# UW-ACL/SCPToolbox.jl

Hardware: NVIDIA H100
Metric: SCP iterations/sec (batch) (higher is better)
Workload: dtype f64

## Files before the change

### scptoolbox.jl_b200/csrc/conic_debug.cu

```cuda
#include "../../include/scpb.h"
#include "conic_symbolic.h"

struct SplitSums {
    std::vector<double> part;
    std::vector<int> cnt, tgt, taken;
    explicit SplitSums(int nslot) : part((size_t)nslot, 0.0), cnt((size_t)nslot, 0), tgt((size_t)nslot, -1), taken((size_t)nslot, 0) {}
    bool add(const int *it, const std::vector<int> &info, double p, double *y)
    {
        if (!it[3]) { y[it[0]] -= p; return true; }
        const size_t q = (size_t)it[3] - 1;
        if (it[3] < 1 || 4 * q + 3 >= info.size()) return false;
        const int *e = &info[4 * q];
        const int sl = e[3];
        if (e[0] != it[0] || e[1] < 0 || e[2] > (int)part.size() || sl < e[1] || sl >= e[2]) return false;
        part[sl] = p;
        if (++cnt[e[1]] == e[2] - e[1]) {
            double acc = y[e[0]];
            for (int k = e[1]; k < e[2]; k++) acc -= part[k];
            y[e[0]] = acc;
            cnt[e[1]] = 0;
        }
        return true;
    }
    bool store(const int *it, double p, double *y)
    {
        if (!it[3]) { y[it[0]] -= p; return true; }
        const int sl = it[3] - 1;
        if (sl < 0 || sl >= (int)part.size() || tgt[sl] >= 0) return false;
        part[sl] = p; tgt[sl] = it[0];
        return true;
    }
    bool take(int t, int s0, int s1, double &acc, bool entry)
    {
        for (int k = s0; k < s1; k++) {
            if (k < 0 || k >= (int)part.size() || tgt[k] != t) return false;
            acc -= part[k];
            taken[k] += entry;
        }
        return true;
    }
    bool level_done()
    {
        bool ok = true;
        for (size_t k = 0; k < cnt.size(); k++) {
            if (cnt[k] || (tgt[k] >= 0 && taken[k] != 1)) ok = false;
            tgt[k] = -1; taken[k] = 0;
        }
        return ok;
    }
};

static bool phase_b_operands(SplitSums &split, const int *it, const int *cm, int nnzL, std::vector<double> &Y, double &e, double &d)
{
    e = Y[it[0]];
    if (!split.take(it[0], cm[0], cm[1], e, true)) return false;
    if (it[3] & 2) { d = e; return true; }
    d = Y[(size_t)nnzL + it[1]];
    if (!split.take(nnzL + it[1], cm[2], cm[3], d, false)) return false;
    Y[it[0]] = e;
    return true;
}

extern "C" int32_t scpb_debug_kkt_solve(int32_t n, int32_t p, int32_t m, const int32_t *A_rp, const int32_t *A_ci,
                                        const int32_t *G_rp, const int32_t *G_ci, int32_t l, int32_t nsoc,
                                        const int32_t *soc_dims, const int32_t *perm, const double *Av,
                                        const double *Gv, const double *wm, double delta, double delta_dyn,
                                        const double *rhs, double *sol, int64_t *info)
{
    ConeSymbolic S;
    static const int zero = 0;
    if (!cone_symbolic_build(S, n, p, m, A_rp, A_ci ? A_ci : &zero, G_rp, G_ci ? G_ci : &zero, l, nsoc, soc_dims, perm))
        return SCPB_ERR_ARG;
    const int nk = S.nk, ntgt = S.nnzL + nk;
    std::vector<double> Y(ntgt), Ls(S.nnzL + 1), invD(nk), v(nk);
    for (int t = 0; t < ntgt; t++) {
        double acc = delta * S.as_sign[t];
        if (S.as_src[t] >= 0) acc += Av[S.as_src[t]];
        for (int k = S.as_ptr[t]; k < S.as_ptr[t + 1]; k++) acc += Gv[S.as_a[k]] * Gv[S.as_b[k]] * wm[S.as_c[k]];
        Y[t] = acc;
    }
    SplitSums split(S.npart);
    int64_t nsplit = 0;
    for (int lv = 0; lv < S.nlevels; lv++) {
        const int R = S.fa_R[lv];
        for (int w = S.fa_lvl[lv]; w < S.fa_lvl[lv + 1]; w++) {
            const int *it = &S.fa_item[4 * (size_t)w];
            if (it[2] - it[1] > R * CONIC_FACTOR_PF) return SCPB_ERR_ARG;
            double part = 0.0;
            for (int k = it[1]; k < it[2]; k++) part += Y[S.ft_op[2 * (size_t)k]] * Ls[S.Lr_pos[S.ft_op[2 * (size_t)k + 1]]];
            if (!split.store(it, part, Y.data())) return SCPB_ERR_ARG;
            nsplit += it[3] != 0;
        }
        for (int w = S.fb_lvl[lv]; w < S.fb_lvl[lv + 1]; w++) {
            const int *it = &S.fb_item[4 * (size_t)w];
            double e, d;
            if (!phase_b_operands(split, it, &S.fb_cmb[4 * (size_t)w], S.nnzL, Y, e, d)) return SCPB_ERR_ARG;
            const double sgn = (it[3] & 1) ? 1.0 : -1.0;
            if (!(sgn * d > delta_dyn)) d = sgn * delta_dyn;
            if (it[3] & 2) invD[it[1]] = 1.0 / d;
            else Ls[it[0]] = e * (1.0 / d);
        }
        if (!split.level_done()) return SCPB_ERR_ARG;
    }
    for (int i = 0; i < nk; i++) v[S.iperm[i]] = rhs[i];
    std::vector<double> Lrow(S.nnzL + 1);
    for (int k = 0; k < S.nnzL; k++) Lrow[k] = Ls[S.Lr_pos[k]];
    for (int lv = 0; lv < S.nlevels; lv++) {
        const int R = S.fwp_R[lv];
        for (int w = S.fwp_lvl[lv]; w < S.fwp_lvl[lv + 1]; w++) {
            const int *it = &S.fwp_item[4 * (size_t)w];
            if (it[2] - it[1] > R * CONIC_SOLVE_PF) return SCPB_ERR_ARG;
            double part = 0.0;
            for (int k = it[1]; k < it[2]; k++) part += Lrow[k] * v[S.Lr_col[k]];
            if (!split.add(it, S.fwc_item, part, v.data())) return SCPB_ERR_ARG;
            nsplit += it[3] != 0;
        }
        if (!split.level_done()) return SCPB_ERR_ARG;
    }
    for (int i = 0; i < nk; i++) v[i] *= invD[i];
    for (int lv = S.nlevels - 1; lv >= 0; lv--) {
        const int R = S.bwp_R[lv];
        for (int w = S.bwp_lvl[lv]; w < S.bwp_lvl[lv + 1]; w++) {
            const int *it = &S.bwp_item[4 * (size_t)w];
            if (it[2] - it[1] > R * CONIC_SOLVE_PF) return SCPB_ERR_ARG;
            double part = 0.0;
            for (int k = it[1]; k < it[2]; k++) part += Ls[k] * v[S.L_ri[k]];
            if (!split.add(it, S.bwc_item, part, v.data())) return SCPB_ERR_ARG;
            nsplit += it[3] != 0;
        }
        if (!split.level_done()) return SCPB_ERR_ARG;
    }
    for (int i = 0; i < nk; i++) sol[i] = v[S.iperm[i]];
    if (info) { info[0] = S.nnzL; info[1] = S.nlevels; info[2] = S.factor_ops; info[3] = (int64_t)S.as_a.size(); info[4] = nsplit; }
    return SCPB_OK;
}

extern "C" int32_t scpb_debug_kkt_solve_sn(int32_t n, int32_t p, int32_t m, const int32_t *A_rp, const int32_t *A_ci,
                                           const int32_t *G_rp, const int32_t *G_ci, int32_t l, int32_t nsoc,
                                           const int32_t *soc_dims, const int32_t *perm, const double *Av,
                                           const double *Gv, const double *wm, double delta, double delta_dyn,
                                           const double *rhs, double *sol, int64_t *info)
{
    ConeSymbolic S;
    static const int zero = 0;
    if (!cone_symbolic_build(S, n, p, m, A_rp, A_ci ? A_ci : &zero, G_rp, G_ci ? G_ci : &zero, l, nsoc, soc_dims, perm))
        return SCPB_ERR_ARG;
    const int nk = S.nk, ntgt = S.nnzL + nk, ns = (int)S.sn_first.size();
    std::vector<double> P((size_t)S.sn_panel_size, 0.0), invD(nk), v(nk);
    for (int t = 0; t < ntgt; t++) {
        double acc = delta * S.as_sign[t];
        if (S.as_src[t] >= 0) acc += Av[S.as_src[t]];
        for (int k = S.as_ptr[t]; k < S.as_ptr[t + 1]; k++) acc += Gv[S.as_a[k]] * Gv[S.as_b[k]] * wm[S.as_c[k]];
        P[(size_t)S.sn_pos_of_target[t]] = acc;
    }
    for (int lv = 0; lv < S.sn_nlevels; lv++)
        for (int w_ = S.sn_lvl_ptr[lv]; w_ < S.sn_lvl_ptr[lv + 1]; w_++) {
            const int s = S.sn_lvl_nodes[w_], a = S.sn_first[s], w = S.sn_width[s], R = S.sn_nrows[s];
            double *Q = &P[(size_t)S.sn_panel_off[s]];
            for (int c = 0; c < w; c++) {
                double d = Q[c + (size_t)R * c];
                const double sgn = (double)S.as_sign[S.nnzL + a + c];
                if (!(sgn * d > delta_dyn)) d = sgn * delta_dyn;
                Q[c + (size_t)R * c] = d;
                invD[a + c] = 1.0 / d;
                for (int r = c + 1; r < R; r++) Q[r + (size_t)R * c] /= d;
                for (int c2 = c + 1; c2 < w; c2++) {
                    const double f = Q[c2 + (size_t)R * c] * d;
                    for (int r = c2; r < R; r++) Q[r + (size_t)R * c2] -= Q[r + (size_t)R * c] * f;
                }
            }
            int k = S.sn_upd_ptr[s];
            for (int y = 0; y < R - w; y++)
                for (int x = y; x < R - w; x++) {
                    double u = 0.0;
                    for (int c = 0; c < w; c++) u += Q[w + x + (size_t)R * c] * Q[c + (size_t)R * c] * Q[w + y + (size_t)R * c];
                    P[(size_t)S.sn_upd_dst[k++]] -= u;
                }
        }
    for (int i = 0; i < nk; i++) v[S.iperm[i]] = rhs[i];
    for (int lv = 0; lv < S.sn_nlevels; lv++)
        for (int w_ = S.sn_lvl_ptr[lv]; w_ < S.sn_lvl_ptr[lv + 1]; w_++) {
            const int s = S.sn_lvl_nodes[w_], w = S.sn_width[s], R = S.sn_nrows[s];
            const double *Q = &P[(size_t)S.sn_panel_off[s]];
            const int *rows = &S.sn_rows[S.sn_rows_ptr[s]];
            for (int c = 0; c < w; c++) {
                const double xc = v[rows[c]];
                for (int r = c + 1; r < R; r++) v[rows[r]] -= Q[r + (size_t)R * c] * xc;
            }
        }
    for (int i = 0; i < nk; i++) v[i] *= invD[i];
    for (int lv = S.sn_nlevels - 1; lv >= 0; lv--)
        for (int w_ = S.sn_lvl_ptr[lv]; w_ < S.sn_lvl_ptr[lv + 1]; w_++) {
            const int s = S.sn_lvl_nodes[w_], w = S.sn_width[s], R = S.sn_nrows[s];
            const double *Q = &P[(size_t)S.sn_panel_off[s]];
            const int *rows = &S.sn_rows[S.sn_rows_ptr[s]];
            for (int c = w - 1; c >= 0; c--) {
                double acc = v[rows[c]];
                for (int r = c + 1; r < R; r++) acc -= Q[r + (size_t)R * c] * v[rows[r]];
                v[rows[c]] = acc;
            }
        }
    for (int i = 0; i < nk; i++) sol[i] = v[S.iperm[i]];
    if (info) {
        info[0] = ns; info[1] = S.sn_nlevels; info[2] = S.sn_panel_size; info[3] = (int64_t)S.sn_upd_dst.size();
        int wmax = 0, rmax = 0;
        for (int s = 0; s < ns; s++) { wmax = std::max(wmax, S.sn_width[s]); rmax = std::max(rmax, S.sn_nrows[s]); }
        info[4] = wmax; info[5] = rmax; info[6] = S.nlevels; info[7] = S.nnzL;
    }
    (void)ns;
    return SCPB_OK;
}

extern "C" int32_t scpb_debug_kkt_solve_hy(int32_t n, int32_t p, int32_t m, const int32_t *A_rp, const int32_t *A_ci,
                                           const int32_t *G_rp, const int32_t *G_ci, int32_t l, int32_t nsoc,
                                           const int32_t *soc_dims, const int32_t *perm, const double *Av,
                                           const double *Gv, const double *wm, double delta, double delta_dyn,
                                           int32_t cut, const double *rhs, double *sol, int64_t *info)
{
    ConeSymbolic S;
    static const int zero = 0;
    if (!cone_symbolic_build(S, n, p, m, A_rp, A_ci ? A_ci : &zero, G_rp, G_ci ? G_ci : &zero, l, nsoc, soc_dims, perm))
        return SCPB_ERR_ARG;
    if (!cone_symbolic_build_hybrid(S, cut)) return SCPB_ERR_UNSUPPORTED;
    const int nk = S.nk, ntgt = S.nnzL + nk, nl = S.hy_nlevels;
    std::vector<double> Y(ntgt), Ls(S.nnzL + 1), invD(nk), v(nk);
    for (int t = 0; t < ntgt; t++) {
        double acc = delta * S.as_sign[t];
        if (S.as_src[t] >= 0) acc += Av[S.as_src[t]];
        for (int k = S.as_ptr[t]; k < S.as_ptr[t + 1]; k++) acc += Gv[S.as_a[k]] * Gv[S.as_b[k]] * wm[S.as_c[k]];
        Y[t] = acc;
    }
    SplitSums split(S.npart);
    for (int lv = 0; lv < nl; lv++) {
        const int R = S.hy_fa_R[lv];
        for (int w = S.hy_fa_lvl[lv]; w < S.hy_fa_lvl[lv + 1]; w++) {
            const int *it = &S.hy_fa_item[4 * (size_t)w];
            if (it[2] - it[1] > R * CONIC_FACTOR_PF) return SCPB_ERR_ARG;
            double part = 0.0;
            for (int k = it[1]; k < it[2]; k++) part += Y[S.hy_ft_op[2 * (size_t)k]] * Ls[S.Lr_pos[S.hy_ft_op[2 * (size_t)k + 1]]];
            if (!split.store(it, part, Y.data())) return SCPB_ERR_ARG;
        }
        for (int w = S.hy_fb_lvl[lv]; w < S.hy_fb_lvl[lv + 1]; w++) {
            const int *it = &S.hy_fb_item[4 * (size_t)w];
            double e, d;
            if (!phase_b_operands(split, it, &S.hy_fb_cmb[4 * (size_t)w], S.nnzL, Y, e, d)) return SCPB_ERR_ARG;
            if (it[3] & 4) continue;
            const double sgn = (it[3] & 1) ? 1.0 : -1.0;
            if (!(sgn * d > delta_dyn)) d = sgn * delta_dyn;
            if (it[3] & 2) invD[it[1]] = 1.0 / d;
            else Ls[it[0]] = e * (1.0 / d);
        }
        if (!split.level_done()) return SCPB_ERR_ARG;
    }
    auto ppos = [&](const int *d, int r, int c) { return r == c ? S.nnzL + d[0] + c : d[3] + c * (d[2] - 1) - (c * (c - 1)) / 2 + (r - c - 1); };
    for (int tl = 0; tl < S.hy_ntl; tl++)
        for (int q = S.hy_tl_ptr[tl]; q < S.hy_tl_ptr[tl + 1]; q++) {
            const int *d = &S.hy_desc[8 * (size_t)q];
            const int w = d[1], R = d[2];
            std::vector<double> Q((size_t)R * w, 0.0), dd(w);
            for (int c = 0; c < w; c++)
                for (int r = c; r < R; r++) Q[r + (size_t)R * c] = Y[ppos(d, r, c)];
            for (int c = 0; c < w; c++) {
                double piv = Q[c + (size_t)R * c];
                const double sgn = ((d[6] >> c) & 1) ? 1.0 : -1.0;
                if (!(sgn * piv > delta_dyn)) piv = sgn * delta_dyn;
                dd[c] = piv;
                invD[d[0] + c] = 1.0 / piv;
                for (int r = c + 1; r < R; r++) Q[r + (size_t)R * c] /= piv;
                for (int c2 = c + 1; c2 < w; c2++) {
                    const double f = Q[c2 + (size_t)R * c] * piv;
                    for (int r = c2; r < R; r++) Q[r + (size_t)R * c2] -= Q[r + (size_t)R * c] * f;
                }
            }
            for (int c = 0; c < w; c++)
                for (int r = c + 1; r < R; r++) Ls[ppos(d, r, c)] = Q[r + (size_t)R * c];
            int k = d[5];
            for (int y = 0; y < R - w; y++)
                for (int x = y; x < R - w; x++) {
                    double u = 0.0;
                    for (int c = 0; c < w; c++) u += Q[w + x + (size_t)R * c] * dd[c] * Q[w + y + (size_t)R * c];
                    Y[S.hy_upd_dst[k++]] -= u;
                }
        }
    for (int i = 0; i < nk; i++) v[S.iperm[i]] = rhs[i];
    std::vector<double> Lrow(S.nnzL + 1);
    for (int k = 0; k < S.nnzL; k++) Lrow[k] = Ls[S.Lr_pos[k]];
// ... 154 lines not shown
```

### scptoolbox.jl_b200/csrc/conic_symbolic.h

```cpp
#pragma once
#include <algorithm>
#include <cstdint>
#include <numeric>
#include <string>
#include <vector>

#ifndef CONIC_FACTOR_PF
#define CONIC_FACTOR_PF 4
#endif
#ifndef CONIC_SOLVE_PF
#define CONIC_SOLVE_PF 4
#endif
#define CONIC_SN_WMAX 8
#define CONIC_SN_RMAX 32
#define CONIC_SN_R1MAX 10
inline int conic_sn_class(int R, int w)
{
    if (w > CONIC_SN_WMAX || R > CONIC_SN_RMAX) return 0;
    if (w == 1 && R <= CONIC_SN_R1MAX) return 1;
    return R <= 8 ? 8 : (R <= 16 ? 16 : 32);
}

struct ConeSymbolic {
    int n = 0, p = 0, m = 0, l = 0, nsoc = 0;
    int nk = 0;
    std::vector<int> soc_dim, soc_off;
    std::vector<int> soc_woff;
    int nwm = 0;
    std::vector<int> A_rp, A_ci, G_rp, G_ci;
    std::vector<int> At_rp, At_ri, At_vi, Gt_rp, Gt_ri, Gt_vi;
    std::vector<int> perm, iperm;
    std::vector<int> L_cp, L_ri;
    std::vector<int> Lr_rp, Lr_pos, Lr_col;
    int nnzL = 0;
    int nlevels = 0;
    std::vector<int> lvl_ptr;
    std::vector<int> lvl_nodes;
    std::vector<int> ft_lvl_ptr;
    std::vector<int> ft_target;
    std::vector<int> ft_op_ptr;
    std::vector<int> ft_op_a, ft_op_b;
    std::vector<int> sc_lvl_ptr, sc_pos, sc_col;
    std::vector<int> as_ptr;
    std::vector<int> as_a, as_b, as_c;
    std::vector<int> as_src;
    std::vector<int> as_sign;
    std::vector<int> fw_item, bw_item;
    std::vector<int> Lr_pc;
    std::vector<int> ft_item;
    std::vector<int> ft_op;
    std::vector<int> sc_item;
    std::vector<int> lvl_maxlen;
    std::vector<int> fwp_item, bwp_item;
    std::vector<int> fwp_lvl, bwp_lvl;
    std::vector<int> fwp_R, bwp_R;
    std::vector<int> fa_item, fa_lvl, fa_R;
    std::vector<int> fb_item, fb_lvl;
    std::vector<int> fc_item, fwc_item, bwc_item;
    std::vector<int> fb_cmb;
    int fslots = 0, sslots = 0;
    int npart = 0;
    std::vector<int> sn_first, sn_width, sn_nrows;
    std::vector<int> sn_rows_ptr, sn_rows;
    std::vector<int> sn_panel_off;
    std::vector<int> sn_lvl_ptr, sn_lvl_nodes;
    std::vector<int> sn_pos_of_target;
    std::vector<int> sn_upd_ptr;
    std::vector<int> sn_upd_dst;
    std::vector<int> sn_upd_xy;
    std::vector<int> sn_sign;
    std::vector<int> sn_cls_ptr;
    int hy_cut = 0, hy_nlevels = 0, hy_ntl = 0;
    std::vector<int> hy_fa_item, hy_fa_lvl, hy_fa_R, hy_fb_item, hy_fb_lvl, hy_ft_op;
    std::vector<int> hy_fwp_item, hy_fwp_lvl, hy_fwp_R, hy_bwp_item, hy_bwp_lvl, hy_bwp_R;
    std::vector<int> hy_fc_item, hy_fwc_item, hy_bwc_item, hy_fb_cmb;
    int hy_fslots = 0, hy_sslots = 0;
    std::vector<int> hy_tl_ptr;
    std::vector<int> hy_desc;
    std::vector<int> hy_upd_dst;
    std::vector<int> hy_is_top;
    bool sn_fits = true;
    long long sn_panel_size = 0;
    int sn_nlevels = 0;
    long long factor_ops = 0;
    std::string err;
};

namespace conic_detail {

inline void number_pieces(std::vector<int> &item, const std::vector<int> &lvl, std::vector<int> &info, int &nslot)
{
    const int nl = (int)lvl.size() - 1;
    info.clear();
    nslot = 0;
    for (int lv = 0; lv < nl; lv++) {
        std::vector<std::pair<int, int>> sp;
        for (int w = lvl[lv]; w < lvl[lv + 1]; w++)
            if (item[4 * (size_t)w + 3]) sp.push_back({item[4 * (size_t)w], w});
        std::stable_sort(sp.begin(), sp.end(), [](const std::pair<int, int> &x, const std::pair<int, int> &y) { return x.first < y.first; });
        int slot = 0;
        for (size_t i = 0; i < sp.size();) {
            size_t j = i;
            while (j < sp.size() && sp[j].first == sp[i].first) j++;
            const int s0 = slot, s1 = slot + (int)(j - i);
            for (; i < j; i++) {
                item[4 * (size_t)sp[i].second + 3] = 1 + (int)(info.size() / 4);
                info.push_back(sp[i].first); info.push_back(s0); info.push_back(s1); info.push_back(slot++);
            }
        }
        nslot = std::max(nslot, slot);
    }
    if (info.empty()) info.assign(4, 0);
}

inline bool combine_in_phase_b(std::vector<int> &fa, const std::vector<int> &fal, const std::vector<int> &info,
                               std::vector<int> &fb, std::vector<int> &fbl, std::vector<int> &cmb, int ntgt, int nnzL,
                               bool extra)
{
    const int nl = (int)fal.size() - 1;
    std::vector<int> nfb, stamp(ntgt, -1), r0(ntgt, 0), r1(ntgt, 0), used(ntgt, 0), entry(ntgt, -1);
    cmb.clear();
    for (int lv = 0; lv < nl; lv++) {
        for (int w = fal[lv]; w < fal[lv + 1]; w++) {
            int *it = &fa[4 * (size_t)w];
            if (it[0] < 0 || it[0] >= ntgt) return false;
            stamp[it[0]] = lv; used[it[0]] = 0;
            if (!it[3]) { r0[it[0]] = r1[it[0]] = 0; continue; }
            const int *e = &info[4 * (size_t)(it[3] - 1)];
            if (e[0] != it[0]) return false;
            r0[it[0]] = e[1]; r1[it[0]] = e[2];
            it[3] = 1 + e[3];
        }
        for (int w = fbl[lv]; w < fbl[lv + 1]; w++) {
            const int *it = &fb[4 * (size_t)w];
            const int t = it[0], pv = nnzL + it[1];
            const bool te = stamp[t] == lv, tp = stamp[pv] == lv;
            for (int q = 0; q < 4; q++) nfb.push_back(it[q]);
            cmb.push_back(te ? r0[t] : 0); cmb.push_back(te ? r1[t] : 0);
            cmb.push_back(tp ? r0[pv] : 0); cmb.push_back(tp ? r1[pv] : 0);
            if (te) { used[t]++; entry[t] = lv; }
        }
        for (int w = fal[lv]; w < fal[lv + 1]; w++) {
            const int t = fa[4 * (size_t)w];
            if (entry[t] == lv) {
                if (used[t] != 1) return false;
                continue;
            }
            if (!extra) return false;
            if (r1[t] > r0[t]) {
                nfb.push_back(t); nfb.push_back(0); nfb.push_back(0); nfb.push_back(4);
                cmb.push_back(r0[t]); cmb.push_back(r1[t]); cmb.push_back(0); cmb.push_back(0);
                used[t] = 1; entry[t] = lv;
            }
        }
        fbl[lv + 1] = (int)(nfb.size() / 4);
    }
    if (nfb.empty()) nfb.assign(4, 0);
    if (cmb.empty()) cmb.assign(4, 0);
    fb.swap(nfb);
    return true;
}

inline void transpose_pattern(int nrow, int ncol, const std::vector<int> &rp, const std::vector<int> &ci,
                              std::vector<int> &t_rp, std::vector<int> &t_ri, std::vector<int> &t_vi)
{
    t_rp.assign(ncol + 1, 0);
    for (int v : ci) t_rp[v + 1]++;
    for (int j = 0; j < ncol; j++) t_rp[j + 1] += t_rp[j];
    t_ri.resize(ci.size());
    t_vi.resize(ci.size());
    std::vector<int> nxt(t_rp.begin(), t_rp.end() - 1);
    for (int r = 0; r < nrow; r++)
        for (int k = rp[r]; k < rp[r + 1]; k++) {
            int q = nxt[ci[k]]++;
            t_ri[q] = r;
            t_vi[q] = k;
        }
}

}

inline bool cone_symbolic_build(ConeSymbolic &S, int n, int p, int m, const int *A_rp, const int *A_ci,
                                const int *G_rp, const int *G_ci, int l, int nsoc, const int *soc_dims,
                                const int *perm_in)
{
    using namespace conic_detail;
    S.n = n; S.p = p; S.m = m; S.l = l; S.nsoc = nsoc; S.nk = n + p;
    const int nk = S.nk;
    S.A_rp.assign(A_rp, A_rp + p + 1);
    S.A_ci.assign(A_ci, A_ci + A_rp[p]);
    S.G_rp.assign(G_rp, G_rp + m + 1);
    S.G_ci.assign(G_ci, G_ci + G_rp[m]);
    S.soc_dim.assign(soc_dims, soc_dims + nsoc);
    S.soc_off.resize(nsoc);
    S.soc_woff.resize(nsoc);
    int off = l, woff = l;
    for (int i = 0; i < nsoc; i++) {
        if (soc_dims[i] < 2) { S.err = "SOC dimension < 2"; return false; }
        S.soc_off[i] = off; S.soc_woff[i] = woff;
        off += soc_dims[i]; woff += soc_dims[i] * soc_dims[i];
    }
    if (off != m) { S.err = "cone dimensions do not sum to m"; return false; }
    S.nwm = woff;
    transpose_pattern(p, n, S.A_rp, S.A_ci, S.At_rp, S.At_ri, S.At_vi);
    transpose_pattern(m, n, S.G_rp, S.G_ci, S.Gt_rp, S.Gt_ri, S.Gt_vi);

    S.perm.resize(nk);
    if (perm_in) S.perm.assign(perm_in, perm_in + nk);
    else std::iota(S.perm.begin(), S.perm.end(), 0);
    S.iperm.assign(nk, -1);
    for (int k = 0; k < nk; k++) {
        int v = S.perm[k];
        if (v < 0 || v >= nk || S.iperm[v] != -1) { S.err = "perm is not a permutation of 0..n+p-1"; return false; }
        S.iperm[v] = k;
    }

    struct Rec { int j, i, a, b, c; };
    std::vector<Rec> recs;
    auto add_block = [&](int r0, int q, int wbase, bool dense) {
        for (int r1 = r0; r1 < r0 + q; r1++)
            for (int r2 = r0; r2 < r0 + q; r2++) {
                if (!dense && r1 != r2) continue;
                const int c = dense ? wbase + (r1 - r0) * q + (r2 - r0) : wbase;
                for (int ka = S.G_rp[r1]; ka < S.G_rp[r1 + 1]; ka++)
                    for (int kb = S.G_rp[r2]; kb < S.G_rp[r2 + 1]; kb++) {
                        const int pi = S.iperm[S.G_ci[ka]], pj = S.iperm[S.G_ci[kb]];
                        if (pi >= pj) recs.push_back({pj, pi, ka, kb, c});
                    }
            }
    };
    for (int r = 0; r < l; r++) add_block(r, 1, r, false);
    for (int i = 0; i < nsoc; i++) add_block(S.soc_off[i], S.soc_dim[i], S.soc_woff[i], true);
    for (int r = 0; r < p; r++)
        for (int k = S.A_rp[r]; k < S.A_rp[r + 1]; k++) {
            int pi = S.iperm[n + r], pj = S.iperm[S.A_ci[k]];
            if (pi < pj) std::swap(pi, pj);
            recs.push_back({pj, pi, -1, k, 0});
        }
    std::sort(recs.begin(), recs.end(), [](const Rec &x, const Rec &y) {
        return x.j != y.j ? x.j < y.j : x.i < y.i;
    });

    std::vector<std::vector<int>> mcol(nk);
    for (const Rec &r : recs)
        if (r.i != r.j && (mcol[r.j].empty() || mcol[r.j].back() != r.i)) mcol[r.j].push_back(r.i);

    std::vector<int> parent(nk, -1);
    std::vector<std::vector<int>> lcol(nk);
    {
        std::vector<std::vector<int>> children(nk);
        std::vector<int> mark(nk, -1);
// ... 56 lines not shown
    std::vector<int> cnt(ntgt, 0);
    S.factor_ops = 0;
    for (int k = 0; k < nk; k++) {
        const int b0 = S.L_cp[k], e0 = S.L_cp[k + 1];
        for (int qa = b0; qa < e0; qa++) {
            cnt[S.nnzL + S.L_ri[qa]]++;
            for (int qb = qa + 1; qb < e0; qb++) {
                int t = lpos(S.L_ri[qb], S.L_ri[qa]);
                if (t < 0) { S.err = "internal: fill entry missing"; return false; }
                cnt[t]++;
            }
        }
    }
    std::vector<long long> optr(ntgt + 1, 0);
    for (int t = 0; t < ntgt; t++) optr[t + 1] = optr[t] + cnt[t];
    S.factor_ops = optr[ntgt];
    if (S.factor_ops > 2000000000LL) { S.err = "factor program too large (bad ordering?)"; return false; }
    std::vector<int> opa(S.factor_ops), opb(S.factor_ops);
    {
        std::vector<long long> nxt(optr.begin(), optr.end() - 1);
        for (int k = 0; k < nk; k++) {
            const int b0 = S.L_cp[k], e0 = S.L_cp[k + 1];
            for (int qa = b0; qa < e0; qa++) {
                long long w = nxt[S.nnzL + S.L_ri[qa]]++;
                opa[w] = qa; opb[w] = qa;
                for (int qb = qa + 1; qb < e0; qb++) {
                    int t = lpos(S.L_ri[qb], S.L_ri[qa]);
                    long long w2 = nxt[t]++;
                    opa[w2] = qb;
                    opb[w2] = qa;
                }
            }
        }
    }
    S.ft_lvl_ptr.assign(S.nlevels + 1, 0);
    S.ft_target.clear(); S.ft_op_ptr.clear(); S.ft_op_a.clear(); S.ft_op_b.clear();
    S.ft_target.reserve(ntgt);
    S.ft_op_a.reserve(S.factor_ops); S.ft_op_b.reserve(S.factor_ops);
    S.sc_lvl_ptr.assign(S.nlevels + 1, 0);
    S.sc_pos.clear(); S.sc_col.clear();
    S.ft_op_ptr.push_back(0);
    for (int lv = 0; lv < S.nlevels; lv++) {
        for (int w = S.lvl_ptr[lv]; w < S.lvl_ptr[lv + 1]; w++) {
            const int j = S.lvl_nodes[w];
            auto emit = [&](int t) {
                S.ft_target.push_back(t);
                for (long long o = optr[t]; o < optr[t + 1]; o++) { S.ft_op_a.push_back(opa[o]); S.ft_op_b.push_back(opb[o]); }
                S.ft_op_ptr.push_back((int)S.ft_op_a.size());
            };
            emit(S.nnzL + j);
            for (int q = S.L_cp[j]; q < S.L_cp[j + 1]; q++) { emit(q); S.sc_pos.push_back(q); S.sc_col.push_back(j); }
        }
        S.ft_lvl_ptr[lv + 1] = (int)S.ft_target.size();
        S.sc_lvl_ptr[lv + 1] = (int)S.sc_pos.size();
    }

    S.as_ptr.assign(ntgt + 1, 0);
    S.as_src.assign(ntgt, -1);
    S.as_sign.assign(ntgt, 0);
    std::vector<int> tcount(ntgt, 0);
    auto tid = [&](int i, int j) { return i == j ? S.nnzL + j : lpos(i, j); };
    for (const Rec &r : recs) {
        int t = tid(r.i, r.j);
        if (t < 0) { S.err = "internal: KKT entry outside L pattern"; return false; }
        if (r.a >= 0) tcount[t]++;
    }
    for (int t = 0; t < ntgt; t++) S.as_ptr[t + 1] = S.as_ptr[t] + tcount[t];
    S.as_a.resize(S.as_ptr[ntgt]); S.as_b.resize(S.as_ptr[ntgt]); S.as_c.resize(S.as_ptr[ntgt]);
    {
        std::vector<int> nxt(S.as_ptr.begin(), S.as_ptr.end() - 1);
        for (const Rec &r : recs) {
            int t = tid(r.i, r.j);
            if (r.a >= 0) { int w = nxt[t]++; S.as_a[w] = r.a; S.as_b[w] = r.b; S.as_c[w] = r.c; }
            else S.as_src[t] = r.b;
        }
    }
    for (int k = 0; k < nk; k++) S.as_sign[S.nnzL + k] = (S.perm[k] < n) ? 1 : -1;

    S.fw_item.resize(4 * (size_t)nk); S.bw_item.resize(4 * (size_t)nk);
    for (int w = 0; w < nk; w++) {
        const int i = S.lvl_nodes[w];
        S.fw_item[4 * w] = i; S.fw_item[4 * w + 1] = S.Lr_rp[i]; S.fw_item[4 * w + 2] = S.Lr_rp[i + 1]; S.fw_item[4 * w + 3] = 0;
        S.bw_item[4 * w] = i; S.bw_item[4 * w + 1] = S.L_cp[i]; S.bw_item[4 * w + 2] = S.L_cp[i + 1]; S.bw_item[4 * w + 3] = 0;
    }
    S.Lr_pc.resize(2 * (size_t)S.nnzL);
    for (int q = 0; q < S.nnzL; q++) { S.Lr_pc[2 * q] = S.Lr_pos[q]; S.Lr_pc[2 * q + 1] = S.Lr_col[q]; }
    const size_t nft = S.ft_target.size();
    S.ft_item.resize(4 * nft);
    for (size_t w = 0; w < nft; w++) {
        const int t = S.ft_target[w];
        S.ft_item[4 * w] = t; S.ft_item[4 * w + 1] = S.ft_op_ptr[w]; S.ft_item[4 * w + 2] = S.ft_op_ptr[w + 1];
        S.ft_item[4 * w + 3] = S.as_sign[t];
    }
    {
        std::vector<int> rowpos(S.nnzL);
        for (int w = 0; w < S.nnzL; w++) rowpos[S.Lr_pos[w]] = w;
        S.sc_item.resize(4 * S.sc_pos.size());
        for (size_t w = 0; w < S.sc_pos.size(); w++) {
            S.sc_item[4 * w] = S.sc_pos[w]; S.sc_item[4 * w + 1] = S.sc_col[w];
            S.sc_item[4 * w + 2] = rowpos[S.sc_pos[w]]; S.sc_item[4 * w + 3] = 0;
        }
    }
    S.lvl_maxlen.assign(3 * (size_t)S.nlevels, 0);
    for (int lv = 0; lv < S.nlevels; lv++) {
        for (int w = S.lvl_ptr[lv]; w < S.lvl_ptr[lv + 1]; w++) {
            const int i = S.lvl_nodes[w];
            S.lvl_maxlen[lv] = std::max(S.lvl_maxlen[lv], S.Lr_rp[i + 1] - S.Lr_rp[i]);
            S.lvl_maxlen[S.nlevels + lv] = std::max(S.lvl_maxlen[S.nlevels + lv], S.L_cp[i + 1] - S.L_cp[i]);
        }
        for (int w = S.ft_lvl_ptr[lv]; w < S.ft_lvl_ptr[lv + 1]; w++)
            S.lvl_maxlen[2 * S.nlevels + lv] = std::max(S.lvl_maxlen[2 * S.nlevels + lv], S.ft_op_ptr[w + 1] - S.ft_op_ptr[w]);
    }
    {
        std::vector<int> rowpos(S.nnzL);
        for (int w = 0; w < S.nnzL; w++) rowpos[S.Lr_pos[w]] = w;
        S.ft_op.resize(2 * S.ft_op_a.size());
        for (size_t k = 0; k < S.ft_op_a.size(); k++) { S.ft_op[2 * k] = S.ft_op_a[k]; S.ft_op[2 * k + 1] = rowpos[S.ft_op_b[k]]; }
    }
    {
        const int PF = CONIC_FACTOR_PF, SLOTS = 512, RMAX = 4;
        S.fa_item.clear(); S.fa_lvl.assign(S.nlevels + 1, 0); S.fa_R.assign(S.nlevels, 1);
        S.fb_item.clear(); S.fb_lvl.assign(S.nlevels + 1, 0);
        std::vector<int> rowpos(S.nnzL);
        for (int w = 0; w < S.nnzL; w++) rowpos[S.Lr_pos[w]] = w;
        for (int lv = 0; lv < S.nlevels; lv++) {
            const int w0 = S.ft_lvl_ptr[lv], w1 = S.ft_lvl_ptr[lv + 1];
            int bestR = 1; long long bestp = -1, bestw = -1;
            for (int R = 1; R <= RMAX; R *= 2) {
                long long items = 0;
                for (int w = w0; w < w1; w++) items += (S.ft_op_ptr[w + 1] - S.ft_op_ptr[w] + R * PF - 1) / (R * PF);
                const long long passes = (items * R + SLOTS - 1) / SLOTS, waste = items * R;
                if (bestp < 0 || passes < bestp || (passes == bestp && waste < bestw)) { bestp = passes; bestw = waste; bestR = R; }
            }
            S.fa_R[lv] = bestR;
            const int cap = bestR * PF;
            for (int w = w0; w < w1; w++) {
                const int k0 = S.ft_op_ptr[w], k1 = S.ft_op_ptr[w + 1], split = (k1 - k0 > cap) ? 1 : 0;
                for (int k = k0; k < k1; k += cap) {
                    S.fa_item.push_back(S.ft_target[w]); S.fa_item.push_back(k);
                    S.fa_item.push_back(std::min(k + cap, k1)); S.fa_item.push_back(split);
                }
            }
            S.fa_lvl[lv + 1] = (int)(S.fa_item.size() / 4);
            for (int w = S.lvl_ptr[lv]; w < S.lvl_ptr[lv + 1]; w++) {
                const int j = S.lvl_nodes[w], pos = (S.as_sign[S.nnzL + j] > 0) ? 1 : 0;
                S.fb_item.push_back(S.nnzL + j); S.fb_item.push_back(j); S.fb_item.push_back(0); S.fb_item.push_back(pos | 2);
                for (int q = S.L_cp[j]; q < S.L_cp[j + 1]; q++) {
                    S.fb_item.push_back(q); S.fb_item.push_back(j); S.fb_item.push_back(rowpos[q]); S.fb_item.push_back(pos);
                }
            }
            S.fb_lvl[lv + 1] = (int)(S.fb_item.size() / 4);
        }
        if (S.fa_item.empty()) S.fa_item.assign(4, 0);
        conic_detail::number_pieces(S.fa_item, S.fa_lvl, S.fc_item, S.fslots);
        if (!conic_detail::combine_in_phase_b(S.fa_item, S.fa_lvl, S.fc_item, S.fb_item, S.fb_lvl, S.fb_cmb, S.nnzL + nk,
                                              S.nnzL, false)) {
            S.err = "internal: a phase-A target of the factorisation is not finished by one phase-B item of its level";
            return false;
        }
    }
    {
        const int ns_max = nk;
        std::vector<int> sn_of(nk, 0);
        S.sn_first.clear(); S.sn_width.clear(); S.sn_nrows.clear();
        for (int j = 0; j < nk;) {
            int k = j;
            while (k + 1 < nk && (k - j + 1) < CONIC_SN_WMAX && S.L_cp[k + 1] > S.L_cp[k] && S.L_ri[S.L_cp[k]] == k + 1 &&
                   (S.L_cp[k + 1] - S.L_cp[k]) == (S.L_cp[k + 2] - S.L_cp[k + 1]) + 1)
                k++;
            const int sid = (int)S.sn_first.size();
            for (int c = j; c <= k; c++) sn_of[c] = sid;
            S.sn_first.push_back(j); S.sn_width.push_back(k - j + 1);
            S.sn_nrows.push_back((k - j + 1) + (S.L_cp[k + 1] - S.L_cp[k]));
            j = k + 1;
        }
        (void)ns_max;
        const int ns = (int)S.sn_first.size();
        S.sn_rows_ptr.assign(ns + 1, 0); S.sn_panel_off.assign(ns + 1, 0);
        for (int s = 0; s < ns; s++) {
            S.sn_rows_ptr[s + 1] = S.sn_rows_ptr[s] + S.sn_nrows[s];
            const long long nxt_ = (long long)S.sn_panel_off[s] + (long long)S.sn_nrows[s] * S.sn_width[s];
            if (nxt_ > 2000000000LL) { S.err = "supernodal panels too large"; return false; }
            S.sn_panel_off[s + 1] = (int)nxt_;
        }
        S.sn_panel_size = S.sn_panel_off[ns];
        S.sn_rows.resize(S.sn_rows_ptr[ns]);
        for (int s = 0; s < ns; s++) {
            const int a = S.sn_first[s], w = S.sn_width[s], b = a + w - 1;
            int o = S.sn_rows_ptr[s];
            for (int c = 0; c < w; c++) S.sn_rows[o++] = a + c;
            for (int q = S.L_cp[b]; q < S.L_cp[b + 1]; q++) S.sn_rows[o++] = S.L_ri[q];
        }
        auto panel_pos = [&](int i, int j) -> int {
            const int s = sn_of[j], a = S.sn_first[s], w = S.sn_width[s], R = S.sn_nrows[s], c = j - a;
            int r;
            if (i < a + w) r = i - a;
            else {
                const int *lo = &S.sn_rows[S.sn_rows_ptr[s] + w], *hi = &S.sn_rows[S.sn_rows_ptr[s] + R];
                const int *it = std::lower_bound(lo, hi, i);
                if (it == hi || *it != i) return -1;
                r = w + (int)(it - lo);
            }
            return S.sn_panel_off[s] + r + R * c;
        };
        S.sn_pos_of_target.assign((size_t)S.nnzL + nk, -1);
        for (int j = 0; j < nk; j++) {
            S.sn_pos_of_target[(size_t)S.nnzL + j] = panel_pos(j, j);
            for (int q = S.L_cp[j]; q < S.L_cp[j + 1]; q++) {
                const int pp = panel_pos(S.L_ri[q], j);
                if (pp < 0) { S.err = "internal: supernode panel does not cover an L entry"; return false; }
                S.sn_pos_of_target[q] = pp;
            }
        }
        S.sn_upd_ptr.assign(ns + 1, 0);
        S.sn_upd_dst.clear(); S.sn_upd_xy.clear();
        S.sn_sign.resize(nk);
        for (int j = 0; j < nk; j++) S.sn_sign[j] = S.as_sign[(size_t)S.nnzL + j];
        for (int s = 0; s < ns; s++) {
            const int w = S.sn_width[s], R = S.sn_nrows[s];
            const int *below = &S.sn_rows[S.sn_rows_ptr[s] + w];
            for (int y = 0; y < R - w; y++)
                for (int x = y; x < R - w; x++) {
                    const int pp = panel_pos(below[x], below[y]);
                    if (pp < 0) { S.err = "internal: supernodal update falls outside the L pattern"; return false; }
                    S.sn_upd_dst.push_back(pp);
                    S.sn_upd_xy.push_back(x | (y << 16));
                }
            if (S.sn_upd_dst.size() > 2000000000ULL) { S.err = "supernodal update lists too large"; return false; }
            S.sn_upd_ptr[s + 1] = (int)S.sn_upd_dst.size();
        }
        std::vector<int> slev(ns, 0);
        for (int s = 0; s < ns; s++) {
            const int b = S.sn_first[s] + S.sn_width[s] - 1;
            if (S.L_cp[b + 1] > S.L_cp[b]) {
                const int ps = sn_of[S.L_ri[S.L_cp[b]]];
                slev[ps] = std::max(slev[ps], slev[s] + 1);
            }
        }
        S.sn_nlevels = 0;
        for (int s = 0; s < ns; s++) S.sn_nlevels = std::max(S.sn_nlevels, slev[s] + 1);
        S.sn_lvl_ptr.assign(S.sn_nlevels + 1, 0);
        for (int s = 0; s < ns; s++) S.sn_lvl_ptr[slev[s] + 1]++;
        for (int l2 = 0; l2 < S.sn_nlevels; l2++) S.sn_lvl_ptr[l2 + 1] += S.sn_lvl_ptr[l2];
        S.sn_lvl_nodes.resize(ns);
        {
            std::vector<int> nxt(S.sn_lvl_ptr.begin(), S.sn_lvl_ptr.end() - 1);
            for (int s = 0; s < ns; s++) S.sn_lvl_nodes[nxt[slev[s]]++] = s;
        }
        auto cls_of = [&](int s) { return conic_sn_class(S.sn_nrows[s], S.sn_width[s]); };
        S.sn_cls_ptr.assign(5 * (size_t)S.sn_nlevels, 0);
        S.sn_fits = true;
        for (int lv = 0; lv < S.sn_nlevels; lv++) {
            int *b = &S.sn_lvl_nodes[S.sn_lvl_ptr[lv]], *e = &S.sn_lvl_nodes[S.sn_lvl_ptr[lv + 1]];
            std::stable_sort(b, e, [&](int x, int y) { int cx = cls_of(x), cy = cls_of(y); return (cx ? cx : 64) < (cy ? cy : 64); });
            int o = S.sn_lvl_ptr[lv];
            S.sn_cls_ptr[5 * lv] = o;
            const int gss[4] = {1, 8, 16, 32};
            for (int q = 0; q < 4; q++) {
                while (o < S.sn_lvl_ptr[lv + 1] && cls_of(S.sn_lvl_nodes[o]) == gss[q]) o++;
                S.sn_cls_ptr[5 * lv + q + 1] = o;
            }
            if (o != S.sn_lvl_ptr[lv + 1]) S.sn_fits = false;
        }
    }
    {
        const int PF = CONIC_SOLVE_PF, SLOTS = 512, RMAX = 4;
        auto build = [&](const std::vector<int> &ptr, std::vector<int> &item, std::vector<int> &lvl, std::vector<int> &Rl) {
            item.clear(); lvl.assign(S.nlevels + 1, 0); Rl.assign(S.nlevels, 1);
            for (int lv = 0; lv < S.nlevels; lv++) {
                int bestR = 1; long long bestp = -1, bestw = -1;
                for (int R = 1; R <= RMAX; R *= 2) {
                    long long items = 0;
                    for (int w = S.lvl_ptr[lv]; w < S.lvl_ptr[lv + 1]; w++) {
                        const int i = S.lvl_nodes[w], len = ptr[i + 1] - ptr[i];
                        items += (len + R * PF - 1) / (R * PF);
                    }
                    const long long passes = (items * R + SLOTS - 1) / SLOTS, waste = items * R;
                    if (bestp < 0 || passes < bestp || (passes == bestp && waste < bestw)) { bestp = passes; bestw = waste; bestR = R; }
                }
                Rl[lv] = bestR;
                const int cap = bestR * PF;
                for (int w = S.lvl_ptr[lv]; w < S.lvl_ptr[lv + 1]; w++) {
                    const int i = S.lvl_nodes[w], k0 = ptr[i], k1 = ptr[i + 1];
                    const int split = (k1 - k0 > cap) ? 1 : 0;
                    for (int k = k0; k < k1; k += cap) {
                        item.push_back(i); item.push_back(k); item.push_back(std::min(k + cap, k1)); item.push_back(split);
                    }
                }
                lvl[lv + 1] = (int)(item.size() / 4);
            }
            if (item.empty()) item.assign(4, 0);
        };
        build(S.Lr_rp, S.fwp_item, S.fwp_lvl, S.fwp_R);
        build(S.L_cp, S.bwp_item, S.bwp_lvl, S.bwp_R);
        int fw_ = 0, bw_ = 0;
        conic_detail::number_pieces(S.fwp_item, S.fwp_lvl, S.fwc_item, fw_);
        conic_detail::number_pieces(S.bwp_item, S.bwp_lvl, S.bwc_item, bw_);
        S.sslots = std::max(fw_, bw_);
    }
    S.npart = std::max(S.fslots, S.sslots);
    return true;
}

inline bool cone_symbolic_build_hybrid(ConeSymbolic &S, int cut)
{
    S.hy_cut = 0; S.hy_nlevels = 0; S.hy_ntl = 0;
    const int nk = S.nk, ns = (int)S.sn_first.size();
// ... 166 lines not shown
```

### scptoolbox.jl_b200/lib.py

```python
from __future__ import annotations

import ctypes as C
import os

import numpy as np

HERE = os.path.dirname(os.path.abspath(__file__))
SO = os.environ.get("SCPB_LIBRARY") or os.path.join(HERE, "libscpb.so")

MODEL_DBLINT, MODEL_ROCKET, MODEL_STARSHIP, MODEL_QUADROTOR, MODEL_FREEFLYER, MODEL_RENDEZVOUS2D = 1, 2, 3, 4, 5, 6
FOH, IMPULSE = 0, 1

_lib = None

_dp = C.POINTER(C.c_double)
_ip = C.POINTER(C.c_int32)

SIGNATURES = {
    "scpb_create": (C.c_int32, [C.c_int32, C.POINTER(C.c_void_p)]),
    "scpb_destroy": (C.c_int32, [C.c_void_p]),
    "scpb_last_error": (C.c_int32, [C.c_void_p, C.c_char_p, C.c_size_t]),
    "scpb_version": (C.c_int32, []),
    "scpb_launch_count": (C.c_int64, [C.c_void_p]),
    "scpb_stream": (C.c_void_p, [C.c_void_p]),
# ... 204 lines not shown
        v = C.c_double(0.0)
        self._check(self.lib.scpb_debug_fp64_peak(self.h, C.byref(v)), "scpb_debug_fp64_peak")
        return v.value

    def debug_constraints(self, t_grid, xd, ud, p, ns, ng):
        xd, pxd = _f64(xd)
        ud, pud = _f64(ud)
        p, pp = _f64(p)
        tg, ptg = _f64(t_grid)
        B, N = xd.shape[0], xd.shape[1]
        assert xd.shape == (B, N, self.nx) and ud.shape == (B, N, self.nu) and p.shape == (B, self.np)
        out = dict(s=np.empty((B, N, ns)), C=np.empty((B, N, ns, self.nx)), D=np.empty((B, N, ns, self.nu)),
                   G=np.empty((B, N, ns, ng)))
        g = lambda k: out[k].ctypes.data_as(_dp)
        rc = self.lib.scpb_debug_constraints(self.h, B, N, ns, ng, ptg, pxd, pud, pp, g("s"), g("C"), g("D"), g("G"))
        self._check(rc, "scpb_debug_constraints")
        return out

    def discretize_dev(self, t_grid, xd, ud, p, iSx_diag, feas_tol, Nsub, A, Bm, Bp, F, r, E, defect, feas,
                       B, N, method=FOH):
        rc = self.lib.scpb_discretize_dev(self.h, method, B, N, Nsub, t_grid, xd, ud, p, iSx_diag,
                                          float(feas_tol), A, Bm, Bp, F, r, E, defect, feas)
        self._check(rc, "scpb_discretize_dev")


def _i32(a):
    a = np.ascontiguousarray(a, dtype=np.int32)
    return a, a.ctypes.data_as(_ip)


class ConeProblem:

    def __init__(self, handle: "Handle", A, G, l: int, soc_dims=(), perm=None):
        self.hd = handle
        self.lib = handle.lib
        self.n, self.p, self.m = A.shape[1], A.shape[0], G.shape[0]
        A = A.tocsr(); G = G.tocsr()
        A.sort_indices(); G.sort_indices()
        self.nnzA, self.nnzG = A.nnz, G.nnz
        self._keep = [_i32(A.indptr), _i32(A.indices), _i32(G.indptr), _i32(G.indices), _i32(list(soc_dims) or [0])]
        pp = None
        if perm is not None:
            self._keep.append(_i32(perm))
            pp = self._keep[-1][1]
        c = C.c_void_p()
        k = self._keep
        rc = self.lib.scpb_cone_setup(handle.h, self.n, self.p, self.m, k[0][1], k[1][1], k[2][1], k[3][1],
                                      int(l), len(soc_dims), k[4][1], pp, C.byref(c))
        handle._check(rc, "scpb_cone_setup")
        self.c = c
        self.l, self.soc_dims = int(l), list(soc_dims)

    def info(self):
        buf = (C.c_int64 * 24)()
        self.lib.scpb_cone_info(self.c, buf)
        keys = ["nk", "nnzL", "levels", "factor_ops", "assembly_ops", "nwm", "group", "capacity"]
        d = dict(zip(keys, [int(v) for v in buf[:8]]))
        d["cycles"] = dict(zip(["equilibrate", "start_point", "residuals", "scale_assemble", "factor", "kkt_solves",
                                "linesearch_update", "total", "ldl_forward", "ldl_backward", "ldl_count",
                                "factor_count"], [int(v) for v in buf[8:20]]))
        d["hybrid"] = dict(zip(["cut_used", "levels", "top_levels", "cut_built"], [int(v) for v in buf[20:24]]))
        fc = d["cycles"]["factor_count"]
        d["cycles"]["factor_count"] = fc & 0xffffffff
        d["cycles"]["factor_retries"] = fc >> 32
        return d

    def ipm_trace(self, rows=256):
        buf = np.zeros((rows, 10))
        n = self.lib.scpb_debug_ipm_trace(self.c, buf.ctypes.data_as(_dp), rows)
        if n <= 0:
            return buf[:0]
        buf = buf[:n]
        return buf[(buf[:, 0] > 0) | (np.arange(n) == 0)]

    def level_profile(self):
        nl = self.info()["levels"]
        buf = (C.c_int64 * (3 * nl))()
        rc = self.lib.scpb_debug_level_profile(self.c, buf, 3 * nl)
        if rc != 0:
            raise ScpbError(f"scpb_debug_level_profile failed ({rc})")
        return np.array(buf[:], dtype=np.int64).reshape(3, nl)

    def close(self):
        if getattr(self, "c", None) is not None and self.c.value:
            self.lib.scpb_cone_free(self.c)
            self.c = C.c_void_p()

    def debug_kkt_solve_dev(self, Avals, Gvals, wm, delta, rhs):
        Avals, pA = _f64(Avals); Gvals, pG = _f64(Gvals); wm, pw = _f64(wm); rhs, pr = _f64(rhs)
        B = rhs.shape[0]
        assert rhs.shape == (B, self.n + self.p)
        sol = np.zeros_like(rhs)
        bad = np.zeros(B, dtype=np.int32)
        rc = self.lib.scpb_debug_kkt_solve_dev(self.c, B, pA, pG, pw, float(delta), pr, sol.ctypes.data_as(_dp),
                                               bad.ctypes.data_as(_ip))
        self.hd._check(rc, "scpb_debug_kkt_solve_dev")
        return sol, bad

    def solve(self, Avals, Gvals, c, b, h, **opts):
        Avals, pA = _f64(Avals); Gvals, pG = _f64(Gvals)
        c, pc = _f64(c); b, pb = _f64(b); h, ph = _f64(h)
        B = c.shape[0]
        assert Avals.shape == (B, self.nnzA) and Gvals.shape == (B, self.nnzG), (Avals.shape, Gvals.shape)
        assert c.shape == (B, self.n) and b.shape == (B, self.p) and h.shape == (B, self.m)
        o = ConeOpts()
        o.nref = -1
        o.equil = -1
        for k_, v in opts.items():
            setattr(o, k_, v)
        out = dict(x=np.empty((B, self.n)), y=np.empty((B, self.p)), z=np.empty((B, self.m)),
                   s=np.empty((B, self.m)), pobj=np.empty(B), dobj=np.empty(B),
                   status=np.zeros(B, dtype=np.int32), iters=np.zeros(B, dtype=np.int32))
        sec = C.c_double(0.0)
        g = lambda k_: out[k_].ctypes.data_as(_dp)
        rc = self.lib.scpb_cone_solve(self.c, B, pA, pG, pc, pb, ph, C.cast(C.byref(o), C.c_void_p), g("x"), g("y"),
                                      g("z"), g("s"), g("pobj"), g("dobj"), out["status"].ctypes.data_as(_ip),
                                      out["iters"].ctypes.data_as(_ip), C.byref(sec))
        self.hd._check(rc, "scpb_cone_solve")
        out["seconds"] = sec.value
        return out


def debug_kkt_solve(A, G, l, soc_dims, perm, Avals, Gvals, wm, delta, rhs, delta_dyn=0.0, supernodal=False, hybrid_cut=0):
    lib = load()
    A = A.tocsr(); G = G.tocsr(); A.sort_indices(); G.sort_indices()
    n, p, m = A.shape[1], A.shape[0], G.shape[0]
    a0, a1, g0, g1 = _i32(A.indptr), _i32(A.indices), _i32(G.indptr), _i32(G.indices)
    sd = _i32(list(soc_dims) or [0])
    pm = _i32(perm) if perm is not None else (None, None)
    Av, pAv = _f64(Avals); Gv, pGv = _f64(Gvals); wmv, pwm = _f64(wm); r, pr = _f64(rhs)
    sol = np.zeros(n + p)
    info = (C.c_int64 * 8)()
    if hybrid_cut > 0:
        rc = lib.scpb_debug_kkt_solve_hy(n, p, m, a0[1], a1[1], g0[1], g1[1], int(l), len(soc_dims), sd[1], pm[1],
                                         pAv, pGv, pwm, float(delta), float(delta_dyn), int(hybrid_cut), pr,
                                         sol.ctypes.data_as(_dp), info)
        if rc != 0:
            raise ScpbError(f"scpb_debug_kkt_solve_hy failed ({rc})")
        keys = ("levels", "top_levels", "top_supernodes", "top_columns", "bridge_factor_items", "bridge_factor_ops",
                "bridge_forward_items", "scalar_levels")
        return sol, dict(zip(keys, [int(v) for v in info]))
    if supernodal:
        rc = lib.scpb_debug_kkt_solve_sn(n, p, m, a0[1], a1[1], g0[1], g1[1], int(l), len(soc_dims), sd[1], pm[1],
                                         pAv, pGv, pwm, float(delta), float(delta_dyn), pr, sol.ctypes.data_as(_dp), info)
        if rc != 0:
            raise ScpbError(f"scpb_debug_kkt_solve_sn failed ({rc})")
        keys = ("supernodes", "sn_levels", "panel_doubles", "update_entries", "max_width", "max_rows", "levels", "nnzL")
        return sol, dict(zip(keys, [int(v) for v in info]))
    rc = lib.scpb_debug_kkt_solve(n, p, m, a0[1], a1[1], g0[1], g1[1], int(l), len(soc_dims), sd[1], pm[1],
                                  pAv, pGv, pwm, float(delta), float(delta_dyn), pr, sol.ctypes.data_as(_dp), info)
    if rc != 0:
        raise ScpbError(f"scpb_debug_kkt_solve failed ({rc})")
    return sol, dict(nnzL=int(info[0]), levels=int(info[1]), factor_ops=int(info[2]), assembly_ops=int(info[3]),
                     split_items=int(info[4]))
```

Baseline: 688.0.

## Route every phase-A factor item of small levels through numbered on-chip slots

During symbolic setup, each level whose phase-A item count fits under a cap (the larger of nk and the widest split count, overridable by an environment variable) is marked on-chip. For those levels every phase-A item, not only the split ones, gets a numbered partial-sum slot. Phase-B then combines them, presumably so the GPU factor kernel can keep partials in shared memory instead of doing scattered global read-modify-writes. The debug path now reports the on-chip level count and counts split items from the combine table. The cost is more slots and more combine work in phase B.

Result: no change. 694.8 (median of 6 runs) (+1.0%).

```diff
diff --git a/scptoolbox.jl_b200/csrc/conic_debug.cu b/scptoolbox.jl_b200/csrc/conic_debug.cu
--- a/scptoolbox.jl_b200/csrc/conic_debug.cu
+++ b/scptoolbox.jl_b200/csrc/conic_debug.cu
@@ -81,6 +81,7 @@
     }
     SplitSums split(S.npart);
     int64_t nsplit = 0;
+    for (size_t q = 0; q + 3 < S.fc_item.size(); q += 4) nsplit += S.fc_item[q + 2] - S.fc_item[q + 1] > 1;
     for (int lv = 0; lv < S.nlevels; lv++) {
         const int R = S.fa_R[lv];
         for (int w = S.fa_lvl[lv]; w < S.fa_lvl[lv + 1]; w++) {
@@ -89,7 +90,6 @@
             double part = 0.0;
             for (int k = it[1]; k < it[2]; k++) part += Y[S.ft_op[2 * (size_t)k]] * Ls[S.Lr_pos[S.ft_op[2 * (size_t)k + 1]]];
             if (!split.store(it, part, Y.data())) return SCPB_ERR_ARG;
-            nsplit += it[3] != 0;
         }
         for (int w = S.fb_lvl[lv]; w < S.fb_lvl[lv + 1]; w++) {
             const int *it = &S.fb_item[4 * (size_t)w];
@@ -131,7 +131,10 @@
         if (!split.level_done()) return SCPB_ERR_ARG;
     }
     for (int i = 0; i < nk; i++) sol[i] = v[S.iperm[i]];
-    if (info) { info[0] = S.nnzL; info[1] = S.nlevels; info[2] = S.factor_ops; info[3] = (int64_t)S.as_a.size(); info[4] = nsplit; }
+    if (info) { info[0] = S.nnzL; info[1] = S.nlevels; info[2] = S.factor_ops; info[3] = (int64_t)S.as_a.size(); info[4] = nsplit;
+        info[5] = 0;
+        for (int v_ : S.fa_onchip) info[5] += v_;
+    }
     return SCPB_OK;
 }
 
diff --git a/scptoolbox.jl_b200/csrc/conic_symbolic.h b/scptoolbox.jl_b200/csrc/conic_symbolic.h
--- a/scptoolbox.jl_b200/csrc/conic_symbolic.h
+++ b/scptoolbox.jl_b200/csrc/conic_symbolic.h
@@ -1,6 +1,7 @@
 #pragma once
 #include <algorithm>
 #include <cstdint>
+#include <cstdlib>
 #include <numeric>
 #include <string>
 #include <vector>
@@ -59,6 +60,7 @@
     std::vector<int> fc_item, fwc_item, bwc_item;
     std::vector<int> fb_cmb;
     int fslots = 0, sslots = 0;
+    std::vector<int> fa_onchip;
     int npart = 0;
     std::vector<int> sn_first, sn_width, sn_nrows;
     std::vector<int> sn_rows_ptr, sn_rows;
@@ -88,15 +90,17 @@
 
 namespace conic_detail {
 
-inline void number_pieces(std::vector<int> &item, const std::vector<int> &lvl, std::vector<int> &info, int &nslot)
+inline void number_pieces(std::vector<int> &item, const std::vector<int> &lvl, std::vector<int> &info, int &nslot,
+                          const std::vector<int> *all = nullptr)
 {
     const int nl = (int)lvl.size() - 1;
     info.clear();
     nslot = 0;
     for (int lv = 0; lv < nl; lv++) {
+        const bool every = all && (*all)[lv];
         std::vector<std::pair<int, int>> sp;
         for (int w = lvl[lv]; w < lvl[lv + 1]; w++)
-            if (item[4 * (size_t)w + 3]) sp.push_back({item[4 * (size_t)w], w});
+            if (every || item[4 * (size_t)w + 3]) sp.push_back({item[4 * (size_t)w], w});
         std::stable_sort(sp.begin(), sp.end(), [](const std::pair<int, int> &x, const std::pair<int, int> &y) { return x.first < y.first; });
         int slot = 0;
         for (size_t i = 0; i < sp.size();) {
@@ -459,7 +463,19 @@
             S.fb_lvl[lv + 1] = (int)(S.fb_item.size() / 4);
         }
         if (S.fa_item.empty()) S.fa_item.assign(4, 0);
-        conic_detail::number_pieces(S.fa_item, S.fa_lvl, S.fc_item, S.fslots);
+        {
+            int split_max = 0;
+            for (int lv = 0; lv < S.nlevels; lv++) {
+                int ns = 0;
+                for (int w = S.fa_lvl[lv]; w < S.fa_lvl[lv + 1]; w++) ns += S.fa_item[4 * (size_t)w + 3] != 0;
+                split_max = std::max(split_max, ns);
+            }
+            int cap = std::max(nk, split_max);
+            if (const char *e = getenv("SCPB_FACTOR_SLOT_CAP")) cap = std::min(cap, atoi(e));
+            S.fa_onchip.assign(S.nlevels, 0);
+            for (int lv = 0; lv < S.nlevels; lv++) S.fa_onchip[lv] = (S.fa_lvl[lv + 1] - S.fa_lvl[lv] <= cap) ? 1 : 0;
+        }
+        conic_detail::number_pieces(S.fa_item, S.fa_lvl, S.fc_item, S.fslots, &S.fa_onchip);
         if (!conic_detail::combine_in_phase_b(S.fa_item, S.fa_lvl, S.fc_item, S.fb_item, S.fb_lvl, S.fb_cmb, S.nnzL + nk,
                                               S.nnzL, false)) {
             S.err = "internal: a phase-A target of the factorisation is not finished by one phase-B item of its level";
diff --git a/scptoolbox.jl_b200/lib.py b/scptoolbox.jl_b200/lib.py
--- a/scptoolbox.jl_b200/lib.py
+++ b/scptoolbox.jl_b200/lib.py
@@ -380,4 +380,4 @@
     if rc != 0:
         raise ScpbError(f"scpb_debug_kkt_solve failed ({rc})")
     return sol, dict(nnzL=int(info[0]), levels=int(info[1]), factor_ops=int(info[2]), assembly_ops=int(info[3]),
-                     split_items=int(info[4]))
+                     split_items=int(info[4]), onchip_levels=int(info[5]))
```
